# zju-vipa/ProtoPFormer

Measured on NVIDIA B200. Metric: prototype_head_train_images_per_sec, higher is better.
Workload: dtype bf16x3 split, fp32 accumulate (fp32-grade)

## Files before the change

include/protohead.h:

```cpp
#ifndef PROTOHEAD_B200_H
#define PROTOHEAD_B200_H

#include <stdint.h>

#ifdef __cplusplus
extern "C" {
#endif

#define PPH_VERSION 202

#define PPH_EINVAL   (-1)
#define PPH_EUNSUP   (-2)
#define PPH_EDRIVER  (-3)

#define PPH_MODE_FP32_FMA 0
#define PPH_MODE_BF16X3   1
#define PPH_MODE_BF16     2

#define PPH_ACT_LOG    0
#define PPH_ACT_LINEAR 1

typedef void* pph_stream_t;

int         pph_version(void);
// ... 63 lines not shown
                  int B, int N, int Din, int D, int K, void* workspace, int parts,
                  float* dWa, float* dba, float* dtokens, pph_stream_t stream);

int pph_loss_tail(const float* logits, const int64_t* labels, const float* ppc_losses,
                  float cov_coe, float mean_coe, float upstream, int B, int C,
                  float* partial, uint32_t* counter, float* out_losses, float* dlogits, pph_stream_t stream);

int pph_loss_combine(const float* ce_losses, const float* ppc_losses, float cov_coe, float mean_coe,
                     float* out_losses, pph_stream_t stream);

#define PPH_FUSE_MEAN 0
#define PPH_FUSE_MAX  1
#define PPH_FUSE_MIN  2
int pph_rollout_ws_bytes(int L, int B, int T, int k_discard, long long* bytes );
int pph_rollout_scores(const float* const* attn_layers , int L, int B, int H, int T,
                       int k_discard, int head_fusion, float identity_w, const float* v0, int drop_first,
                       void* workspace, float* scores, int K, int32_t* idx32, int64_t* idx64, pph_stream_t stream);

int pph_adamw_step(int n_seg, float* const* params, const float* const* grads, float* const* exp_avg,
                   float* const* exp_avg_sq, const long long* numel , const int* group ,
                   const float* hyper, double beta1, double beta2, float eps, float grad_scale,
                   int* step_state, pph_stream_t stream);

int pph_rollout_cls_rows(const float* const* cls_layers , int n_cls, int B, int H,
                         int Tc, int k_discard, int head_fusion, float identity_w, float* v0, pph_stream_t stream);

int pph_class_maps(const float* Zs, const float* z2s, const float* Pl, const float* p2l,
                   const int32_t* idx32, const int64_t* labels, int B, int K, int D, int P, int m, int N,
                   int act_fn, float eps, float* maps, pph_stream_t stream);


int pph_head_prep_supported(int B, int N, int Din, int D, int K);
int pph_head_prep(const float* scores, const float* tokens, const float* Wa, const float* ba,
                  int B, int H, int N, int Din, int D, int K, float center,
                  int32_t* idx32, int64_t* idx64,
                  float* Zs, float* Zc, float* z2s, float* z2c, float* z2s_ctr, float* z2c_ctr,
                  float* z2s_hi, float* z2c_hi, uint16_t* Zs_hi, uint16_t* Zs_lo, uint16_t* Zc_hi, uint16_t* Zc_lo,
                  const float* Pl, int P, uint16_t* Pl_hi, uint16_t* Pl_lo, float* p2l, float* p2l_ctr, float* p2l_hi,
                  const float* Pgl, int Pg, uint16_t* Pg_hi, uint16_t* Pg_lo, float* p2g, float* p2g_ctr, float* p2g_hi,
                  pph_stream_t stream);

int pph_head_mid_ws_bytes(int B, int K, int D, int P, int Pg, int C, int m, long long* bytes );
int pph_head_mid(const float* act_l, const float* act_g, const float* dmin_l, const float* dmin_g,
                 const int32_t* argmin_l, const float* Wl, const float* Wg, const int64_t* labels,
                 int B, int K, int D, int P, int Pg, int C, int m, int N,
                 float global_coe, int act_fn, float eps, float upstream, int train,
                 int use_ppc, const float* Zs, const float* z2s, const float* Pl, const float* p2l,
                 const int32_t* idx32, float cov_thresh, float mean_thresh, float cov_coe, float mean_coe,
                 void* workspace, void* bwd_workspace,
                 float* logits, float* logits_g, float* logits_l, float* losses, float* dlogits,
                 float* g_l, float* g_g, float* pairT, float* dZs_ppc, float* dP_img,
                 float* losses_mirror ,
                 pph_stream_t stream);

#define PPH_BWD2_TOKENS 1
#define PPH_BWD2_PROTOS 2
#define PPH_BWD2_CLS    4
int pph_similarity_bwd2_supported(int B, int K, int D, int P, int Pg);
int pph_similarity_bwd2_ws_bytes(int B, int K, int D, int P, long long* bytes );
int pph_similarity_bwd2(int parts, const float* g_l, const float* g_g, const float* pairT, void* bwd_workspace,
                        const float* Zs, const float* Zc, const float* Pl, const float* Pgl,
                        int B, int K, int D, int P, int Pg, int m,
                        const float* add_dZs, const float* dP_img, int dpre_out,
                        float* dZs, float* dZc, float* dPl, float* dPg, pph_stream_t stream);

int pph_similarity_bwd_fused(int parts ,
                             const float* g_l, const float* g_g, const int32_t* argmin_l,
                             const float* Zs, const float* Zc, const float* Pl, const float* Pgl,
                             int B, int K, int D, int P, int Pg, int m, void* workspace, void* step_workspace,
                             const float* add_dZs, const float* dP_img, int dpre_out,
                             float* dZs, float* dZc, float* dPl, float* dPg, pph_stream_t stream);

int pph_addon_bwd2_supported(int B, int N, int Din, int D, int K);
int pph_addon_bwd2_ws_bytes(int B, int N, int Din, int D, int K, long long* bytes );
int pph_addon_bwd2(int parts, const float* tokens, const int32_t* idx32, const float* Wa,
                   const float* dpre_s, const float* dpre_c,
                   int B, int N, int Din, int D, int K, void* workspace,
                   float* dWa, float* dba, float* dtokens, pph_stream_t stream);

int pph_addon_tc2_supported(int B, int N, int Din, int D, int K);
int pph_addon_tc2_ws_bytes(int B, int N, int Din, int D, int K, long long* bytes );
int pph_addon_fwd2(const float* tokens, const int32_t* idx32, const float* Wa, const float* ba,
                   int B, int N, int Din, int D, int K,
                   float* Zs, float* Zc, float* z2s, float* z2c,
                   float center, float* z2s_ctr, float* z2c_ctr, float* z2s_hi, float* z2c_hi,
                   uint16_t* Zs_hi, uint16_t* Zs_lo, uint16_t* Zc_hi, uint16_t* Zc_lo,
                   void* workspace, pph_stream_t stream);
int pph_select_addon_fwd(const float* scores , int H, const float* tokens, const float* Wa, const float* ba,
                         int B, int N, int Din, int D, int K, int32_t* idx32 ,
                         float* Zs, float* Zc, float* z2s, float* z2c,
                         float center, float* z2s_ctr, float* z2c_ctr, float* z2s_hi, float* z2c_hi,
                         uint16_t* Zs_hi, uint16_t* Zs_lo, uint16_t* Zc_hi, uint16_t* Zc_lo,
                         void* workspace, pph_stream_t stream);
int pph_addon_bwd3(int parts, const float* tokens, const int32_t* idx32, const float* Wa,
                   const float* dpre_s, const float* dpre_c, const float* dpre_add_s ,
                   int B, int N, int Din, int D, int K, void* workspace,
                   float* dWa, float* dba, float* dtokens, pph_stream_t stream);

int pph_ppc_dense_fwd(const float* act, const int32_t* idx32, const int64_t* labels, int B, int P, int K, int m, int N,
                      float cov_thresh, float mean_thresh, float* stats, float* partial, unsigned int* counter,
                      float* losses, pph_stream_t stream);
int pph_ppc_dense_bwd(const float* act, const int32_t* idx32, const int64_t* labels, const float* stats,
                      const float* g_cov, const float* g_mean, int B, int P, int K, int m, int N, float mean_thresh,
                      float* dact, pph_stream_t stream);

int pph_gather_rows_host(const float* tokens_host, const int32_t* idx32, int B, int N, int Din, int K,
// ... 12 lines not shown
```

protopformer_b200/_lib.py:

```python
from __future__ import annotations

import ctypes as C
import os

import torch

_HERE = os.path.dirname(os.path.abspath(__file__))
LIB_PATH = os.path.join(_HERE, "lib", "libprotohead_b200.so")

MODE_FP32_FMA, MODE_BF16X3, MODE_BF16 = 0, 1, 2
MODES = {"fp32_fma": MODE_FP32_FMA, "fp32": MODE_BF16X3, "bf16x3": MODE_BF16X3, "bf16": MODE_BF16}
ACT_LOG, ACT_LINEAR = 0, 1
ACTS = {"log": ACT_LOG, "linear": ACT_LINEAR}

_p, _i, _f = C.c_void_p, C.c_int, C.c_float

SIGNATURES = {
    "pph_version": [],
    "pph_last_error_string": [],
    "pph_sm_count": [],
    "pph_set_option": [C.c_char_p, _i],
    "pph_select_topk": [_p, _i, _i, _i, _i, _p, _p, _p],
    "pph_addon_fwd": [_p, _p, _p, _p, _i, _i, _i, _i, _i, _p, _p, _p, _p, _f, _p, _p, _p, _p, _p, _p, _p, _p, _p],
    "pph_split_rows": [_p, _i, _i, _f, _p, _p, _p, _p, _p, _p],
    "pph_similarity_fwd": [_i, _i, _f, _i, _i, _i, _i, _i] + [_p] * 24,
    "pph_similarity_plan": [_i, _i, _i, _i, _i, _i, _i, C.POINTER(C.c_int), C.POINTER(C.c_int)],
    "pph_logits_fwd": [_p, _p, _p, _p, _i, _i, _i, _i, _f, _p, _p, _p, _p],
    "pph_ppc_fwd": [_p, _p, _p, _p, _p, _p, _i, _i, _i, _i, _i, _i, _i, _f, _f, _f, _p, _p, _p, _p, _p, _p],
    "pph_ppc_bwd": [_p, _p, _p, _p, _p, _p, _p, _f, _f, _i, _i, _i, _i, _i, _i, _i, _f, _f, _f, _i, _p, _p, _p],
    "pph_logits_bwd": [_p, _p, _p, _p, _p, _p, _p, _i, _i, _i, _i, _f, _i, _f, _p, _p, _p],
    "pph_similarity_bwd_ws_bytes": [_i, _i, _i, _i, _i, C.POINTER(C.c_longlong)],
    "pph_similarity_bwd": [_p, _p, _p, _p, _p, _p, _p, _i, _i, _i, _i, _i, _p, _i, _p, _p, _p, _p, _p, _p, _p],
    "pph_loss_tail": [_p, _p, _p, _f, _f, _f, _i, _i, _p, _p, _p, _p, _p],
    "pph_loss_combine": [_p, _p, _f, _f, _p, _p],
    "pph_rollout_ws_bytes": [_i, _i, _i, _i, C.POINTER(C.c_longlong)],
    "pph_rollout_scores": [_p, _i, _i, _i, _i, _i, _i, _f, _p, _i, _p, _p, _i, _p, _p, _p],
    "pph_adamw_step": [_i, _p, _p, _p, _p, _p, _p, _p, C.c_double, C.c_double, _f, _f, _p, _p],
    "pph_rollout_cls_rows": [_p, _i, _i, _i, _i, _i, _i, _f, _p, _p],
    "pph_class_maps": [_p, _p, _p, _p, _p, _p, _i, _i, _i, _i, _i, _i, _i, _f, _p, _p],
    "pph_addon_bwd_ws_bytes": [_i, _i, _i, _i, _i, C.POINTER(C.c_longlong)],
    "pph_addon_bwd": [_p, _p, _p, _p, _p, _p, _p, _i, _i, _i, _i, _i, _p, _i, _p, _p, _p, _p],
    "pph_head_prep_supported": [_i, _i, _i, _i, _i],
    "pph_head_prep": [_p, _p, _p, _p, _i, _i, _i, _i, _i, _i, _f] + [_p] * 14 + [_p, _i, _p, _p, _p, _p, _p] * 2 + [_p],
    "pph_head_mid_ws_bytes": [_i, _i, _i, _i, _i, _i, _i, C.POINTER(C.c_longlong)],
    "pph_head_mid": [_p] * 8 + [_i] * 8 + [_f, _i, _f, _f, _i, _i] + [_p] * 5 + [_f] * 4 + [_p] * 14,
    "pph_similarity_bwd2_supported": [_i, _i, _i, _i, _i],
    "pph_similarity_bwd2_ws_bytes": [_i, _i, _i, _i, C.POINTER(C.c_longlong)],
    "pph_similarity_bwd2": [_i] + [_p] * 8 + [_i] * 6 + [_p, _p, _i] + [_p] * 5,
    "pph_addon_bwd2_supported": [_i, _i, _i, _i, _i],
    "pph_addon_bwd2_ws_bytes": [_i, _i, _i, _i, _i, C.POINTER(C.c_longlong)],
    "pph_addon_bwd2": [_i] + [_p] * 5 + [_i] * 5 + [_p] * 5,
    "pph_similarity_bwd_fused": [_i] + [_p] * 7 + [_i] * 6 + [_p, _p, _p, _p, _i] + [_p] * 5,
    "pph_addon_tc2_supported": [_i, _i, _i, _i, _i],
    "pph_addon_tc2_ws_bytes": [_i, _i, _i, _i, _i, C.POINTER(C.c_longlong)],
    "pph_addon_fwd2": [_p, _p, _p, _p, _i, _i, _i, _i, _i, _p, _p, _p, _p, _f] + [_p] * 10,
    "pph_addon_bwd3": [_i] + [_p] * 6 + [_i] * 5 + [_p] * 5,
    "pph_select_addon_fwd": [_p, _i, _p, _p, _p, _i, _i, _i, _i, _i, _p, _p, _p, _p, _p, _f] + [_p] * 10,
    "pph_ppc_dense_fwd": [_p, _p, _p, _i, _i, _i, _i, _i, _f, _f, _p, _p, _p, _p, _p],
    "pph_ppc_dense_bwd": [_p, _p, _p, _p, _p, _p, _i, _i, _i, _i, _i, _f, _p, _p],
    "pph_gather_rows_host": [_p, _p, _i, _i, _i, _i, _p, _i, _p],
    "pph_peer_flag_bytes": [C.POINTER(C.c_longlong)],
    "pph_peer_allreduce": [_p, C.c_ulonglong, C.c_longlong, _i, _i, C.c_longlong, C.c_longlong, _i, _i, _p],
}
_RESTYPES = {"pph_last_error_string": C.c_char_p}

KERNELS_PER_CALL = {
    "pph_select_topk": 1, "pph_addon_fwd": 1, "pph_split_rows": 1, "pph_logits_fwd": 1, "pph_ppc_fwd": 1,
    "pph_ppc_bwd": 1, "pph_logits_bwd": 1, "pph_similarity_bwd": 2, "pph_addon_bwd": 3, "pph_loss_tail": 1, "pph_loss_combine": 1, "pph_rollout_scores": 2, "pph_adamw_step": 1, "pph_class_maps": 1, "pph_rollout_cls_rows": 1,
    "pph_head_prep": 1, "pph_head_mid": 1, "pph_similarity_bwd_fused": 1, "pph_addon_bwd2": 1, "pph_addon_fwd2": 1,
    "pph_peer_allreduce": 1, "pph_gather_rows_host": 1,
    "pph_ppc_dense_fwd": 1, "pph_ppc_dense_bwd": 1, "pph_select_addon_fwd": 1,
}

_ENV_OPTIONS = {"PPH_PDL": "pdl", "PPH_SIM_LANES": "sim_lanes", "PPH_SIM_SHARED": "sim_shared", "PPH_SIM_EPI": "sim_epi",
                "PPH_ROLLOUT": "rollout", "PPH_CLASSMAP": "classmap", "PPH_DEBUG": "debug",
                "PPH_LOGITS_BWD": "logits_bwd", "PPH_GATHER": "gather"}

_lib = None
_launches = 0


def launch_count() -> int:
    return _launches


def load() -> C.CDLL:
    global _lib
    if _lib is None:
        if not os.path.exists(LIB_PATH):
            raise RuntimeError(
                f"{LIB_PATH} is missing: build it with `python -m protopformer_b200.build` "
                "(needs nvcc; there is no CPU or PyTorch fallback for the prototype head)")
        lib = C.CDLL(LIB_PATH)
        for name, args in SIGNATURES.items():
            fn = getattr(lib, name)
            fn.argtypes = args
            fn.restype = _RESTYPES.get(name, C.c_int)
        for env, opt in _ENV_OPTIONS.items():
            v = os.environ.get(env)
            if v is not None and v.strip() != "":
                if lib.pph_set_option(opt.encode(), int(v)) != 0:
                    raise RuntimeError(f"{env}: {lib.pph_last_error_string().decode()}")
        _lib = lib
    return _lib


_DTYPES = (torch.float32, torch.int32, torch.int64, torch.bfloat16, torch.uint8, torch.int8, torch.uint16, torch.int16)


def _ptr(t):
    if t is None:
        return None
    assert t.is_cuda, "prototype-head tensors must live on a CUDA device (no CPU path exists)"
    assert t.is_contiguous(), "prototype-head tensors must be contiguous"
    assert t.dtype in _DTYPES, f"prototype-head entry points do not take {t.dtype} tensors (cast to float32 first)"
    return t.data_ptr()


def _stream():
    return torch.cuda.current_stream().cuda_stream


# ... 22 lines not shown
```

protopformer_b200/csrc/pph_mid.cu:

```cuda
#include <math.h>

#include "pph_bins.cuh"
#include "pph_common.cuh"
#include "pph_step2.cuh"

namespace pph {

constexpr int kMidThreads = 256;
constexpr int kMidTB = 64;
constexpr int kMidPS = 32;
constexpr int kMidAST = 68;

struct MidArgs {
    int B, Bp, K, D, P, Pg, C, Cp, m, N, side;
    int tiles_b, S_l, S_g, nsl_l, nsl_g;
    int n_ll, n_bin, n_ppc, n_cls_cta;
    int have_ppc;
    int ppc_dpre;
    float gc, eps, upstream, cov_thresh, mean_thresh, cov_coe, mean_coe;
    int act_fn, train;
    const float *act_l, *act_g, *dmin_l, *dmin_g;
    const int32_t* argmin_l;
    const float *Wl, *Wg;
    const int64_t* labels;
    float *logits, *logits_g, *logits_l, *losses, *dlogits, *g_l, *g_g;
    float* losses_mirror;
    float2* pairT;
    float *part, *dlT, *ce_part, *ppc_part, *ppc_losses;
    unsigned int* ctr;
    int32_t *bin_start, *item_start, *bin_list;
    int4* item_desc;
    int32_t *cls_id, *cls_start, *cls_item, *cls_order;
    const float *Zs, *z2s, *Pl, *p2l;
    const int32_t* idx;
    float *dZs_ppc, *dP_img;
};

__device__ __forceinline__ float block_sum_any(float v, float* red, int nwarp) {
    v = warp_sum(v);
    const int lane = threadIdx.x & 31, warp = threadIdx.x >> 5;
    __syncthreads();
    if (lane == 0) red[warp] = v;
    __syncthreads();
    float s = 0.f;
    for (int w = 0; w < nwarp; ++w) s += red[w];
    return s;
}

__device__ __forceinline__ float block_sum_mid(float v, float* red) {
    v = warp_sum(v);
    const int lane = threadIdx.x & 31, warp = threadIdx.x >> 5;
    __syncthreads();
    if (lane == 0) red[warp] = v;
    __syncthreads();
    float s = 0.f;
#pragma unroll
    for (int w = 0; w < kMidThreads / 32; ++w) s += red[w];
    return s;
}

__device__ __forceinline__ void write_total(const MidArgs& a) {
    const float ce = __ldcg(a.losses + 1);
    const float cov = a.have_ppc ? __ldcg(a.ppc_losses) : 0.f, mean = a.have_ppc ? __ldcg(a.ppc_losses + 1) : 0.f;
    const float total = ce + a.cov_coe * cov + a.mean_coe * mean;
    a.losses[0] = total;
    a.losses[2] = cov;
    a.losses[3] = mean;
    if (a.losses_mirror) {
        *reinterpret_cast<float4*>(a.losses_mirror) = make_float4(total, ce, cov, mean);
        __threadfence_system();
    }
}
__device__ __forceinline__ void role_finished(const MidArgs& a) {
    if (!a.have_ppc) {
        write_total(a);
        return;
    }
    __threadfence();
    if (atomicAdd(a.ctr + 2, 1u) == 1u) {
        __threadfence();
        write_total(a);
        a.ctr[2] = 0u;
// ... 182 lines not shown
        }
        cp_async_commit();
        const bool keepW = nsl <= Sg;
        const float coef = glob ? a.gc : 1.0f - a.gc;
        const float* dmin = glob ? a.dmin_g : a.dmin_l;
        float* gout = glob ? a.g_g : a.g_l;
        for (int sl = sg; sl < nsl; sl += Sg) {
            const int p0 = sl * kMidPS;
            if (!keepW) {
                __syncthreads();
                stage_w(Ws, W, np, p0, C, WST);
                cp_async_commit();
            }
            cp_async_wait<0>();
            __syncthreads();
            float g8[8];
#pragma unroll
            for (int i = 0; i < 8; ++i) g8[i] = 0.f;
#pragma unroll 4
            for (int c = 0; c < C; ++c) {
                const float4 d0 = *reinterpret_cast<const float4*>(&dls[c * kMidAST + warp * 8]);
                const float4 d1 = *reinterpret_cast<const float4*>(&dls[c * kMidAST + warp * 8 + 4]);
                const float w = Ws[lane * WST + c];
                g8[0] = fmaf(d0.x, w, g8[0]); g8[1] = fmaf(d0.y, w, g8[1]); g8[2] = fmaf(d0.z, w, g8[2]); g8[3] = fmaf(d0.w, w, g8[3]);
                g8[4] = fmaf(d1.x, w, g8[4]); g8[5] = fmaf(d1.y, w, g8[5]); g8[6] = fmaf(d1.z, w, g8[6]); g8[7] = fmaf(d1.w, w, g8[7]);
            }
            const int p = p0 + lane;
            if (p < np) {
                float2 pr[8];
#pragma unroll
                for (int i = 0; i < 8; ++i) {
                    const int b = b0 + warp * 8 + i;
                    float g = 0.f;
                    int am = 0;
                    if (b < B) {
                        const size_t o = (size_t)b * np + p;
                        g = coef * g8[i] * dact_of_dist(__ldg(dmin + o), a.act_fn, a.eps);
                        gout[o] = g;
                        am = glob ? a.K : __ldg(a.argmin_l + o);
                    }
                    pr[i] = make_float2(g, __int_as_float(am));
                }
                if (a.pairT) {
                    float4* dst = reinterpret_cast<float4*>(a.pairT + (size_t)(glob ? a.P + p : p) * a.Bp + b0 + warp * 8);
#pragma unroll
                    for (int i = 0; i < 4; ++i) dst[i] = make_float4(pr[2 * i].x, pr[2 * i].y, pr[2 * i + 1].x, pr[2 * i + 1].y);
                }
            }
        }
    }
    grid_finish(a.ctr, a.ctr + 1, (unsigned int)a.n_ll);
}

__device__ __forceinline__ void ppc_role(const MidArgs& a, int b, int part, int nsplit, float* sm) {
    const int nthr = blockDim.x;
    const int K = a.K, D = a.D, m = a.m, B = a.B, side = a.side;
    const int zs = D + 4;
    float* Prow = sm;
    float* Zt = Prow + m * D;
    float* dsl = Zt + (size_t)K * zs;
    float* wbuf = dsl + m * K;
    float* st = wbuf + m * K;
    float* red = st + m * 8;
    const int tid = threadIdx.x, lane = tid & 31, warp = tid >> 5, nwarp = nthr >> 5;
    long y = a.labels[b];
    if (y < 0) y = 0;
    if (y * m + m > a.P) y = a.P / m - 1;
    const int prow0 = (int)y * m;
    for (int i = tid; i < m * D / 4; i += nthr) cp_async16(Prow + 4 * i, a.Pl + (size_t)prow0 * D + 4 * i);
    const float* Zb = a.Zs + (size_t)b * K * D;
    {
        const int d4 = D >> 2;
        for (int r = warp; r < K; r += nwarp)
            for (int c = lane; c < d4; c += 32) cp_async16(Zt + (size_t)r * zs + 4 * c, Zb + (size_t)r * D + 4 * c);
    }
    cp_async_commit();
    cp_async_wait<0>();
    __syncthreads();
    const int JG = K * m <= nthr ? m : (K * 5 <= nthr ? 5 : (K * 3 <= nthr ? 3 : (K * 2 <= nthr ? 2 : 1)));
    for (int t = tid; t < K * JG; t += nthr) {
        const int r = t % K, jg = t / K;
        const float4* zr = reinterpret_cast<const float4*>(Zt + (size_t)r * zs);
        const float zz = __ldg(a.z2s + (size_t)b * K + r);
        for (int j = jg; j < m; j += JG) {
            const float4* pr = reinterpret_cast<const float4*>(Prow + (size_t)j * D);
            float a0 = 0.f, a1 = 0.f, a2 = 0.f, a3 = 0.f;
#pragma unroll 4
            for (int c = 0; c < D / 4; ++c) {
                const float4 z = zr[c], p = pr[c];
                a0 = fmaf(z.x, p.x, a0); a1 = fmaf(z.y, p.y, a1); a2 = fmaf(z.z, p.z, a2); a3 = fmaf(z.w, p.w, a3);
            }
            const float dot = (a0 + a1) + (a2 + a3);
            const float d = relu_keep_nan(zz + fmaf(-2.0f, dot, __ldg(a.p2l + prow0 + j)));
            dsl[j * K + r] = d;
            wbuf[j * K + r] = act_of_dist(d, a.act_fn, a.eps);
        }
    }
    __syncthreads();
    float cov_sum = 0.f;
    const float scale = (float)a.N / (float)(a.N - 1);
    for (int j = warp; j < m; j += nwarp) {
        float S = 0.f, Sr = 0.f, Sc = 0.f;
        for (int k = lane; k < K; k += 32) {
            const float w = wbuf[j * K + k];
            const int n = __ldg(a.idx + (size_t)b * K + k);
            S += w;
// ... 75 lines not shown
        const float dw = (dV * ((dr * dr - Vr) + (dc * dc - Vc)) + st[j * 8 + 6] * dr + st[j * 8 + 7] * dc) / S;
        const float d = dsl[j * K + r];
        dsl[j * K + r] = 2.0f * dw * dact_of_dist(d, a.act_fn, a.eps);
    }
    __syncthreads();
    const int ngrp = (D + 127) >> 7;
    for (int r = warp * nsplit + part; r < K; r += nwarp * nsplit) {
        float S = 0.f;
        for (int j = 0; j < m; ++j) S += dsl[j * K + r];
        float* out = a.dZs_ppc + ((size_t)b * K + r) * D;
        for (int g = 0; g < ngrp; ++g) {
            const int d = g * 128 + lane * 4;
            if (d >= D) continue;
            const float4 z = *reinterpret_cast<const float4*>(Zt + (size_t)r * zs + d);
            float4 acc = make_float4(z.x * S, z.y * S, z.z * S, z.w * S);
#pragma unroll 2
            for (int j = 0; j < m; ++j) {
                const float c = -dsl[j * K + r];
                const float4 p = *reinterpret_cast<const float4*>(Prow + j * D + d);
                acc.x = fmaf(c, p.x, acc.x); acc.y = fmaf(c, p.y, acc.y); acc.z = fmaf(c, p.z, acc.z); acc.w = fmaf(c, p.w, acc.w);
            }
            if (a.ppc_dpre) {
                acc.x *= z.x * (1.0f - z.x); acc.y *= z.y * (1.0f - z.y); acc.z *= z.z * (1.0f - z.z); acc.w *= z.w * (1.0f - z.w);
            }
            *reinterpret_cast<float4*>(out + d) = acc;
        }
    }
    for (int it = warp * nsplit + part; it < m * ngrp; it += nwarp * nsplit) {
        const int j = it / ngrp, g = it - j * ngrp;
        const int d = g * 128 + lane * 4;
        if (d >= D) continue;
        float S = 0.f;
        float4 acc = make_float4(0.f, 0.f, 0.f, 0.f);
#pragma unroll 4
        for (int r = 0; r < K; ++r) {
            const float c = dsl[j * K + r];
            const float4 z = *reinterpret_cast<const float4*>(Zt + (size_t)r * zs + d);
            S += c;
            acc.x = fmaf(c, z.x, acc.x); acc.y = fmaf(c, z.y, acc.y); acc.z = fmaf(c, z.z, acc.z); acc.w = fmaf(c, z.w, acc.w);
        }
        const float4 p = *reinterpret_cast<const float4*>(Prow + j * D + d);
        *reinterpret_cast<float4*>(a.dP_img + ((size_t)b * m + j) * D + d) =
            make_float4(p.x * S - acc.x, p.y * S - acc.y, p.z * S - acc.z, p.w * S - acc.w);
    }
}

template <int CJ>
__global__ void __launch_bounds__(kMidThreads)
head_mid_kernel(const MidArgs a) {
    pdl_sync();
    extern __shared__ __align__(16) float sm_mid[];
    const int bid = blockIdx.x;
    if (bid < a.n_ll) {
        ll_role<CJ>(a, sm_mid);
    } else if (bid < a.n_ll + a.n_bin) {
        bin_tokens_body<false>(bid - a.n_ll, a.argmin_l, a.K, a.P, a.bin_start, a.item_start, a.bin_list,
                        reinterpret_cast<int*>(sm_mid), a.item_desc);
    } else if (bid < a.n_ll + a.n_bin + a.n_ppc) {
        ppc_role(a, bid - a.n_ll - a.n_bin, 0, 1, sm_mid);
    } else {
        const int n_cls = a.P / a.m;
        for (int b = threadIdx.x; b < a.B; b += kMidThreads) {
            long y = a.labels[b];
            if (y < 0) y = 0;
            if (y * a.m + a.m > a.P) y = a.P / a.m - 1;
            a.cls_id[b] = (int)y;
        }
        __threadfence();
        __syncthreads();
        bin_tokens_body<true>(0, a.cls_id, n_cls, a.B, a.cls_start, a.cls_item, a.cls_order, reinterpret_cast<int*>(sm_mid));
    }
}

constexpr int kPpcSplit = 2, kPpcThreads = 512;
__global__ void __launch_bounds__(kPpcThreads)
head_ppc_kernel(const MidArgs a) {
    pdl_sync();
    extern __shared__ __align__(16) float sm_mid[];
    ppc_role(a, blockIdx.x / kPpcSplit, blockIdx.x % kPpcSplit, kPpcSplit, sm_mid);
}

struct MidPlan {
    int tiles_b, nsl_l, nsl_g, S_l, S_g, n_ll, Cp, Bp;
    size_t smem_ll, smem_ppc, smem_bin;
};

static MidPlan mid_plan(int B, int K, int D, int P, int Pg, int C, int m, int max_ctas) {
    MidPlan p;
    p.tiles_b = ceil_div(B, kMidTB);
    p.nsl_l = ceil_div(P, kMidPS);
    p.nsl_g = Pg > 0 ? ceil_div(Pg, kMidPS) : 0;
    p.Cp = (C + 3) & ~3;
    p.Bp = p.tiles_b * kMidTB;
    int budget = max_ctas / p.tiles_b;
    const int need = Pg > 0 ? 2 : 1;
    if (budget < need) budget = need;
    if (p.nsl_l + p.nsl_g <= budget) {
        p.S_l = p.nsl_l;
        p.S_g = p.nsl_g;
    } else if (Pg > 0) {
        p.S_l = (int)((long)budget * p.nsl_l / (p.nsl_l + p.nsl_g));
        if (p.S_l < 1) p.S_l = 1;
        if (p.S_l > budget - 1) p.S_l = budget - 1;
        p.S_g = budget - p.S_l;
        if (p.S_l > p.nsl_l) p.S_l = p.nsl_l;
        if (p.S_g > p.nsl_g) p.S_g = p.nsl_g;
    } else {
        p.S_l = budget < p.nsl_l ? budget : p.nsl_l;
        p.S_g = 0;
    }
    p.n_ll = p.tiles_b * (p.S_l + p.S_g);
    const int WST = C | 1;
    p.smem_ll = sizeof(float) * ((size_t)kMidPS * WST + (size_t)kMidPS * kMidAST + (size_t)C * kMidAST + 2 * 4 * 64 * 4 + 3 * 256 + 8);
    p.smem_ppc = sizeof(float) * ((size_t)m * D + (size_t)K * (D + 4) + 2 * (size_t)m * K + 8 * (size_t)m + 32);
    p.smem_bin = bin_tokens_smem_bytes(K);
    return p;
}

struct MidWs {
    unsigned int* ctr;
    float *part, *dlT, *ce_part, *ppc_part, *ppc_losses;
    size_t bytes;
};

static MidWs mid_carve(void* base, const MidPlan& p, int B) {
    MidWs w;
    char* q = static_cast<char*>(base);
    size_t off = 0;
    auto take = [&](size_t n) { char* r = q ? q + off : nullptr; off += (n + 255) / 256 * 256; return r; };
    w.ctr = reinterpret_cast<unsigned int*>(take(sizeof(int) * 8));
    w.ppc_losses = reinterpret_cast<float*>(take(sizeof(float) * 2));
    w.ce_part = reinterpret_cast<float*>(take(sizeof(float) * (size_t)B));
    w.ppc_part = reinterpret_cast<float*>(take(sizeof(float) * 2 * (size_t)B));
    w.dlT = reinterpret_cast<float*>(take(sizeof(float) * (size_t)p.Cp * p.Bp));
    w.part = reinterpret_cast<float*>(take(sizeof(float) * (size_t)(p.S_l + p.S_g) * B * p.Cp));
    w.bytes = off + 256;
    return w;
}

static int mid_max_ctas() {
    int n = pph_sm_count();
    return n > 0 ? n : 148;
}

}

extern "C" int pph_head_mid_ws_bytes(int B, int K, int D, int P, int Pg, int C, int m, long long* bytes) {
    using namespace pph;
    PPH_REQUIRE(bytes && B >= 1 && K >= 1 && D >= 1 && P >= 1 && Pg >= 0 && C >= 1 && m >= 1, PPH_EINVAL,
                "pph_head_mid_ws_bytes: bad args");
    const MidPlan p = mid_plan(B, K, D, P, Pg, C, m, 1 << 20);
    *bytes = (long long)mid_carve(nullptr, p, B).bytes;
    return 0;
}

extern "C" int pph_head_mid(const float* act_l, const float* act_g, const float* dmin_l, const float* dmin_g,
                            const int32_t* argmin_l, const float* Wl, const float* Wg, const int64_t* labels,
                            int B, int K, int D, int P, int Pg, int C, int m, int N,
                            float global_coe, int act_fn, float eps, float upstream, int train,
                            int use_ppc, const float* Zs, const float* z2s, const float* Pl, const float* p2l,
                            const int32_t* idx32, float cov_thresh, float mean_thresh, float cov_coe, float mean_coe,
                            void* workspace, void* bwd_workspace,
                            float* logits, float* logits_g, float* logits_l, float* losses, float* dlogits,
                            float* g_l, float* g_g, float* pairT, float* dZs_ppc, float* dP_img,
                            float* losses_mirror, pph_stream_t stream) {
    using namespace pph;
    PPH_REQUIRE(act_l && dmin_l && Wl && labels && workspace && logits && logits_g && logits_l && losses, PPH_EINVAL,
                "pph_head_mid: null pointer");
    PPH_REQUIRE(Pg == 0 || (act_g && dmin_g && Wg), PPH_EINVAL, "pph_head_mid: null global-branch pointer");
    PPH_REQUIRE((reinterpret_cast<uintptr_t>(losses_mirror) & 15) == 0, PPH_EINVAL, "pph_head_mid: losses_mirror must be 16-byte aligned");
    PPH_REQUIRE(B >= 1 && K >= 1 && D >= 4 && P >= 1 && Pg >= 0 && C >= 1 && m >= 1 && N >= 2, PPH_EINVAL,
                "pph_head_mid: bad dims");
    PPH_REQUIRE(C <= 256, PPH_EUNSUP, "pph_head_mid: C=%d > 256 (use the modular entry points)", C);
    PPH_REQUIRE(!train || (argmin_l && dlogits && g_l && bwd_workspace && (Pg == 0 || g_g)), PPH_EINVAL,
                "pph_head_mid: null training pointer");
    PPH_REQUIRE(!use_ppc || (Zs && z2s && Pl && p2l && idx32 && (!train || (dZs_ppc && dP_img))), PPH_EINVAL,
                "pph_head_mid: null PPC pointer");
    const int max_ctas = mid_max_ctas();
    const MidPlan p = mid_plan(B, K, D, P, Pg, C, m, max_ctas);
    const MidWs w = mid_carve(workspace, p, B);
    MidArgs a;
    a.B = B; a.Bp = p.Bp; a.K = K; a.D = D; a.P = P; a.Pg = Pg; a.C = C; a.Cp = p.Cp; a.m = m; a.N = N;
    a.side = (int)lrint(sqrt((double)N));
    a.tiles_b = p.tiles_b; a.S_l = p.S_l; a.S_g = p.S_g; a.nsl_l = p.nsl_l; a.nsl_g = p.nsl_g;
    a.ppc_dpre = (use_ppc & 4) ? 1 : 0;
    use_ppc &= 3;
    const bool have_ppc = use_ppc != 0, run_ll = use_ppc != 3, run_ppc = use_ppc == 1 || use_ppc == 3;
    a.have_ppc = have_ppc ? 1 : 0;
    a.n_ll = run_ll ? p.n_ll : 0;
    a.n_bin = (train && run_ll) ? B : 0;
    a.n_ppc = run_ppc ? B : 0;
    a.gc = global_coe; a.eps = eps; a.upstream = upstream; a.cov_thresh = cov_thresh; a.mean_thresh = mean_thresh;
    a.cov_coe = cov_coe; a.mean_coe = mean_coe; a.act_fn = act_fn; a.train = train;
    a.act_l = act_l; a.act_g = act_g; a.dmin_l = dmin_l; a.dmin_g = dmin_g; a.argmin_l = argmin_l;
    a.Wl = Wl; a.Wg = Wg; a.labels = labels;
    a.logits = logits; a.logits_g = logits_g; a.logits_l = logits_l; a.losses = losses; a.dlogits = dlogits;
    a.losses_mirror = losses_mirror;
    a.g_l = g_l; a.g_g = g_g; a.pairT = reinterpret_cast<float2*>(pairT);
    a.part = w.part; a.dlT = w.dlT; a.ce_part = w.ce_part; a.ppc_part = w.ppc_part; a.ppc_losses = w.ppc_losses;
    a.ctr = w.ctr;
    a.bin_start = a.item_start = a.bin_list = nullptr;
    a.item_desc = nullptr;
    a.cls_id = a.cls_start = a.cls_item = a.cls_order = nullptr;
    a.n_cls_cta = 0;
    if (train) {
        const Step2Bins bw = carve_bins(bwd_workspace, B, K, P);
        a.bin_start = bw.bin_start; a.item_start = bw.item_start; a.bin_list = bw.bin_list;
        a.item_desc = bw.item_desc;
        a.cls_id = bw.cls_id; a.cls_start = bw.cls_start; a.cls_item = bw.cls_item; a.cls_order = bw.cls_order;
        if (have_ppc && run_ll && bin_tokens_smem_bytes(P / m) <= 200 * 1024) a.n_cls_cta = 1;
    }
    a.Zs = Zs; a.z2s = z2s; a.Pl = Pl; a.p2l = p2l; a.idx = idx32; a.dZs_ppc = dZs_ppc; a.dP_img = dP_img;
    size_t smem = run_ll ? p.smem_ll : 0;
    if (a.n_bin && p.smem_bin > smem) smem = p.smem_bin;
    if (a.n_cls_cta && bin_tokens_smem_bytes(P / m) > smem) smem = bin_tokens_smem_bytes(P / m);
    if (have_ppc) {
        PPH_REQUIRE(D % 4 == 0 && a.side * a.side == N && P >= m && m <= kMidThreads, PPH_EINVAL, "pph_head_mid: bad PPC dims");
        PPH_REQUIRE(p.smem_ppc <= 200 * 1024, PPH_EUNSUP, "pph_head_mid: an image's K x D slice does not fit shared memory");
        if (run_ppc && p.smem_ppc > smem) smem = p.smem_ppc;
    }
    PPH_REQUIRE(smem <= 220 * 1024, PPH_EUNSUP, "pph_head_mid: shared memory %zu B", smem);
    PPH_REQUIRE(p.n_ll <= max_ctas, PPH_EUNSUP, "pph_head_mid: B=%d needs %d co-resident CTAs (> %d SMs)", B, p.n_ll,
                max_ctas);
    if (use_ppc == 3) {
        cudaError_t e = opt_in_smem(head_ppc_kernel, (int)p.smem_ppc);
        if (e != cudaSuccess) { set_error("pph_head_mid: %s", cudaGetErrorString(e)); return (int)e; }
        launch_k(head_ppc_kernel, dim3(B * kPpcSplit), dim3(kPpcThreads), p.smem_ppc, as_stream(stream), a);
        return launch_status("pph_head_mid(ppc)");
    }
    const int cj = ceil_div(C, 32);
    PPH_REQUIRE(!(have_ppc && train && run_ll) || a.n_cls_cta == 1, PPH_EUNSUP, "pph_head_mid: too many classes");

    const dim3 grid(a.n_ll + a.n_bin + a.n_ppc + a.n_cls_cta), block(kMidThreads);
    cudaStream_t st = as_stream(stream);
#define PPH_MID(CJ)                                                                                                   \
    do {                                                                                                              \
        cudaError_t e = opt_in_smem(head_mid_kernel<CJ>, (int)smem); \
        if (e != cudaSuccess) { set_error("pph_head_mid: %s", cudaGetErrorString(e)); return (int)e; }                \
        launch_k(head_mid_kernel<CJ>, grid, block, smem, st, a);                                                      \
    } while (0)
    if (cj <= 4) PPH_MID(4);
    else if (cj <= 7) PPH_MID(7);
    else PPH_MID(8);
#undef PPH_MID
    return launch_status("pph_head_mid");
}
```

protopformer_b200/ops.py:

```python
from __future__ import annotations

import dataclasses
import math

import torch

from . import _lib


@dataclasses.dataclass(frozen=True)
class HeadConfig:

    K: int
    global_coe: float = 0.5
    act_fn: str = "log"
    eps: float = 1e-4
    mode: str = "fp32"
    ppc_cov_thresh: float = 1.0
    ppc_mean_thresh: float = 2.0
    center: float = 0.5

    @property
    def mode_id(self) -> int:
        return _lib.MODES[self.mode]
# ... 593 lines not shown

class FusedHeadStep:

    def __init__(self, cfg: HeadConfig, B, N, Din, D, P, Pg, C, m, device, heads: int = 0, ppc_cov_coe: float = 0.1,
                 ppc_mean_coe: float = 0.5, train: bool = True, use_ppc: bool = True, schedule=None, variants=None):
        if not fused_step_supported(B, N, Din, D, cfg.K, P, Pg, C, m):
            raise ValueError("shape outside FusedHeadStep's kernels: use FusedHeadStepV1")
        self.cfg, self.train, self.use_ppc = cfg, train, use_ppc
        tc_bits = _lib.load().pph_addon_tc2_supported(B, N, Din, D, cfg.K)
        tc1_ok = Din % 8 == 0 and D % 8 == 0 and cfg.mode_id != _lib.MODE_FP32_FMA
        v = {"prep": "tc" if (tc_bits & 1) else ("tc1" if tc1_ok else "simt"),
             "addon_bwd": "tc" if (tc_bits & 6) == 6 else "simt", "bwd": "gather", "ppc": "late",
             "select": "fused" if (tc_bits & 8) else "kernel"}
        v.update(variants or {})
        if v["select"] == "fused" and not (tc_bits & 8):
            v["select"] = "kernel"
        if v["prep"] == "tc" and not (tc_bits & 1):
            v["prep"] = "tc1" if tc1_ok else "simt"
        if v["prep"] == "tc1" and not tc1_ok:
            v["prep"] = "simt"
        if v["addon_bwd"] == "tc" and (tc_bits & 6) != 6:
            v["addon_bwd"] = "simt"
        if v["bwd"] == "staged" and not _lib.load().pph_similarity_bwd2_supported(B, cfg.K, D, P, Pg):
            v["bwd"] = "gather"
        self.variants = v
        self.stop_after = 0
        self.dims = (B, N, Din, D, P, Pg, C, m, heads)
        self.cov_coe, self.mean_coe = float(ppc_cov_coe), float(ppc_mean_coe)
        K = cfg.K
        f32, bf, i32 = torch.float32, torch.bfloat16, torch.int32
        e = lambda *s, dt=f32: torch.empty(s, dtype=dt, device=device)
        self.split = cfg.mode_id != _lib.MODE_FP32_FMA
        self.idx32 = e(B, K, dt=i32)
        self.Zs, self.Zc, self.z2s, self.z2c = e(B, K, D), e(B, D), e(B, K), e(B)
        names = ("z2s_ctr", "z2c_ctr", "z2s_hi", "z2c_hi", "Zs_hi", "Zs_lo", "Zc_hi", "Zc_lo", "P_hi", "P_lo", "Pg_hi",
                 "Pg_lo", "p2_ctr", "p2_hi", "pg2_ctr", "pg2_hi")
        if self.split:
            shapes = ((B, K), (B,), (B, K), (B,), (B * K, D), (B * K, D), (B, D), (B, D), (P, D), (P, D), (Pg, D), (Pg, D),
                      (P,), (P,), (Pg,), (Pg,))
            for n, sh in zip(names, shapes):
                setattr(self, n, e(*sh, dt=bf if ("_hi" in n or "_lo" in n) and n[0] in "ZP" else f32))
        else:
            for n in names:
                setattr(self, n, None)
        self.p2, self.pg2 = e(P), e(Pg)
        self.dmin_l, self.act_l, self.argmin = e(B, P), e(B, P), e(B, P, dt=i32)
        self.dmin_g, self.act_g = e(B, Pg), e(B, Pg)
        self.logits, self.logits_g, self.logits_l = e(B, C), e(B, C), e(B, C)
        self.losses = torch.zeros(4, dtype=f32, device=device)
        self.ws_mid = _ws("pph_head_mid_ws_bytes", B, K, D, P, Pg, C, m, zero=True, device=device)
        self.ws_tc = _ws("pph_addon_tc2_ws_bytes", B, N, Din, D, K, zero=True, device=device)
        self.side = torch.cuda.Stream(device=device)
        self.side2 = torch.cuda.Stream(device=device)
        self.ev = [torch.cuda.Event() for _ in range(8)]
        self.dlogits = self.g_l = self.g_g = self.pairT = self.ws_bins = None
        self.dZs_ppc = self.dP_img = None
        if train:
            Bp = (B + 63) // 64 * 64
            self.dlogits, self.g_l, self.g_g = e(B, C), e(B, P), e(B, Pg)
            self.pairT = e(P + Pg, Bp, 2)
            self.ws_bins = _ws("pph_similarity_bwd2_ws_bytes", B, K, D, P, zero=True, device=device)
            self.ws_gather = bwd_workspace(B, K, D, P, Pg, device)
            if use_ppc:
                self.dZs_ppc, self.dP_img = e(B, K, D), e(B, m, D)
            self.dZs, self.dZc = e(B, K, D), e(B, D)
            self.dtokens = e(B, 1 + N, Din)
            self.ws_addon = _ws("pph_addon_bwd2_ws_bytes", B, N, Din, D, K, zero=True, device=device)
            if self.variants["addon_bwd"] == "tc":
                self.dtokens.zero_()


    def step(self, tokens, scores, labels, Wa, ba, P, Pg, Wl, Wg, grads=None, upstream: float = 1.0, reduce_hook=None,
             idx32=None, loss_mirror=None):
        own_idx = self.idx32
        sel_idx = own_idx if idx32 is None else idx32
        B, N, Din, D, Pn, Pgn, C, m, H = self.dims
        cfg, K = self.cfg, self.cfg.K
        c = _lib.call
        main, side, side2, ev = torch.cuda.current_stream(), self.side, self.side2, self.ev
        hook = reduce_hook or (lambda which: None)
        if self.variants["prep"] in ("tc", "tc1"):
            ev[3].record(main)
            side.wait_event(ev[3])
            with torch.cuda.stream(side):
                c("pph_split_rows", P, Pn, D, float(cfg.center), self.P_hi, self.P_lo, self.p2, self.p2_ctr, self.p2_hi)
                c("pph_split_rows", Pg, Pgn, D, float(cfg.center), self.Pg_hi, self.Pg_lo, self.pg2, self.pg2_ctr, self.pg2_hi)
                if self.train and self.variants["addon_bwd"] == "tc":
                    self.dtokens.zero_()
                ev[4].record(side)
            if self.variants["prep"] == "tc1":
                if idx32 is None:
                    c("pph_select_topk", scores, B, max(H, 1), N, K, sel_idx, None)
                c("pph_addon_fwd", tokens, sel_idx, Wa, ba, B, N, Din, D, K, self.Zs, self.Zc, self.z2s, self.z2c,
                  float(cfg.center), self.z2s_ctr, self.z2c_ctr, self.z2s_hi, self.z2c_hi, self.Zs_hi, self.Zs_lo,
                  self.Zc_hi, self.Zc_lo)
            elif idx32 is None and self.variants["select"] == "fused":
                c("pph_select_addon_fwd", scores, max(H, 1), tokens, Wa, ba, B, N, Din, D, K, sel_idx, self.Zs, self.Zc,
                  self.z2s, self.z2c, float(cfg.center), self.z2s_ctr, self.z2c_ctr, self.z2s_hi, self.z2c_hi, self.Zs_hi,
                  self.Zs_lo, self.Zc_hi, self.Zc_lo, self.ws_tc)
            else:
                if idx32 is None:
                    c("pph_select_topk", scores, B, max(H, 1), N, K, sel_idx, None)
                c("pph_addon_fwd2", tokens, sel_idx, Wa, ba, B, N, Din, D, K, self.Zs, self.Zc, self.z2s, self.z2c,
                  float(cfg.center), self.z2s_ctr, self.z2c_ctr, self.z2s_hi, self.z2c_hi, self.Zs_hi, self.Zs_lo,
                  self.Zc_hi, self.Zc_lo, self.ws_tc)
            main.wait_event(ev[4])
        else:
            if self.train and self.variants["addon_bwd"] == "tc":
                ev[3].record(main)
                side.wait_event(ev[3])
                with torch.cuda.stream(side):
                    self.dtokens.zero_()
                    ev[4].record(side)
            c("pph_head_prep", scores, tokens, Wa, ba, B, max(H, 1), N, Din, D, K, float(cfg.center), sel_idx, None,
              self.Zs, self.Zc, self.z2s, self.z2c, self.z2s_ctr, self.z2c_ctr, self.z2s_hi, self.z2c_hi,
              self.Zs_hi, self.Zs_lo, self.Zc_hi, self.Zc_lo,
              P, Pn, self.P_hi, self.P_lo, self.p2, self.p2_ctr, self.p2_hi,
              Pg, Pgn, self.Pg_hi, self.Pg_lo, self.pg2, self.pg2_ctr, self.pg2_hi)
            if self.train and self.variants["addon_bwd"] == "tc":
                main.wait_event(ev[4])
        if self.stop_after == 1:
            return self.losses
        mode = cfg.mode_id
        sel = {_lib.MODE_FP32_FMA: 0, _lib.MODE_BF16X3: 1, _lib.MODE_BF16: 2}[mode]
        c("pph_similarity_fwd", mode, cfg.act_id, float(cfg.eps), B, K, D, Pn, Pgn, self.Zs, self.Zc,
          (self.z2s, self.z2s_ctr, self.z2s_hi)[sel], (self.z2c, self.z2c_ctr, self.z2c_hi)[sel],
          self.Zs_hi, self.Zs_lo, self.Zc_hi, self.Zc_lo, P, Pg,
          (self.p2, self.p2_ctr, self.p2_hi)[sel], (self.pg2, self.pg2_ctr, self.pg2_hi)[sel],
          self.P_hi, self.P_lo, self.Pg_hi, self.Pg_lo,
          self.dmin_l, self.argmin, self.act_l, self.dmin_g, self.act_g, None, None)
        if self.stop_after == 2:
            return self.losses
        ppc = self.use_ppc and self.train
        vr = self.variants
        late = ppc and vr["ppc"] == "late" and vr["bwd"] == "gather" and vr["addon_bwd"] == "tc"
        split_ppc = ppc and (vr["ppc"] == "split" or late)

        def mid(use_ppc):
            c("pph_head_mid", self.act_l, self.act_g, self.dmin_l, self.dmin_g, self.argmin, Wl, Wg, labels,
              B, K, D, Pn, Pgn, C, m, N, float(cfg.global_coe), cfg.act_id, float(cfg.eps), float(upstream),
              1 if self.train else 0, use_ppc, self.Zs, self.z2s, P, self.p2, sel_idx,
              float(cfg.ppc_cov_thresh), float(cfg.ppc_mean_thresh), self.cov_coe, self.mean_coe,
              self.ws_mid, self.ws_bins, self.logits, self.logits_g, self.logits_l, self.losses, self.dlogits,
              self.g_l, self.g_g, self.pairT if vr["bwd"] == "staged" else None, self.dZs_ppc if ppc else None,
              self.dP_img if ppc else None, loss_mirror)

        if split_ppc:
            ev[0].record(main)
            side.wait_event(ev[0])
            with torch.cuda.stream(side):
                mid(3 + (4 if late else 0))
                ev[6 if late else 1].record(side)
            mid(2)
            if not late:
                main.wait_event(ev[1])
        else:
            mid(1 if ppc else 0)
        if not self.train or self.stop_after == 3:
            if late:
                main.wait_event(ev[6])
            return self.losses

        def gather(parts, add, dpi):
            c("pph_similarity_bwd_fused", parts, self.g_l, self.g_g, self.argmin, self.Zs, self.Zc, P, Pg, B, K, D, Pn, Pgn,
              m, self.ws_gather, self.ws_bins, add, dpi, 1, self.dZs, self.dZc, grads["P"], grads["Pg"])

        dpre_add = None
        if late:
            gather(3, None, None)
            ev[2].record(main)
            with torch.cuda.stream(side):
                side.wait_event(ev[2])
                gather(4, None, self.dP_img)
                hook("protos")
                ev[1].record(side)
            dpre_add = self.dZs_ppc
        elif vr["bwd"] == "gather":
            gather(3, self.dZs_ppc if ppc else None, self.dP_img if ppc else None)
            hook("protos")
            ev[1].record(main)
        else:
            bwd = lambda parts: c("pph_similarity_bwd2", parts, self.g_l, self.g_g, self.pairT, self.ws_bins, self.Zs,
                                  self.Zc, P, Pg, B, K, D, Pn, Pgn, m, self.dZs_ppc if ppc else None,
# ... 48 lines not shown
```

Measured before the change: 428,200.

## Detect class-structured last layer and use closed-form logits and grads

Adds a kernel on the side stream that checks, on every call, whether each last-layer weight matrix takes only two values: one for a prototype's own class and another everywhere else. When both matrices match, the mid kernel's logits role computes logits as a per-class sum plus a total sum, and computes prototype gradients in closed form instead of through the general matrix path. Otherwise it falls back to the existing role. The check costs an extra kernel launch, a full read of the weights and an event wait before the mid stage, and it only pays off when the weights keep this structure.

```diff
diff --git a/include/protohead.h b/include/protohead.h
--- a/include/protohead.h
+++ b/include/protohead.h
@@ -139,6 +139,9 @@
                  float* g_l, float* g_g, float* pairT, float* dZs_ppc, float* dP_img,
                  float* losses_mirror ,
                  pph_stream_t stream);
+
+#define PPH_LL_PATTERN_BYTES 32
+int pph_last_layer_pattern(const float* Wl, int P, const float* Wg, int Pg, int C, void* workspace, pph_stream_t stream);
 
 #define PPH_BWD2_TOKENS 1
 #define PPH_BWD2_PROTOS 2
diff --git a/protopformer_b200/_lib.py b/protopformer_b200/_lib.py
--- a/protopformer_b200/_lib.py
+++ b/protopformer_b200/_lib.py
@@ -44,6 +44,7 @@
     "pph_head_prep": [_p, _p, _p, _p, _i, _i, _i, _i, _i, _i, _f] + [_p] * 14 + [_p, _i, _p, _p, _p, _p, _p] * 2 + [_p],
     "pph_head_mid_ws_bytes": [_i, _i, _i, _i, _i, _i, _i, C.POINTER(C.c_longlong)],
     "pph_head_mid": [_p] * 8 + [_i] * 8 + [_f, _i, _f, _f, _i, _i] + [_p] * 5 + [_f] * 4 + [_p] * 14,
+    "pph_last_layer_pattern": [_p, _i, _p, _i, _i, _p, _p],
     "pph_similarity_bwd2_supported": [_i, _i, _i, _i, _i],
     "pph_similarity_bwd2_ws_bytes": [_i, _i, _i, _i, C.POINTER(C.c_longlong)],
     "pph_similarity_bwd2": [_i] + [_p] * 8 + [_i] * 6 + [_p, _p, _i] + [_p] * 5,
@@ -67,7 +68,7 @@
 KERNELS_PER_CALL = {
     "pph_select_topk": 1, "pph_addon_fwd": 1, "pph_split_rows": 1, "pph_logits_fwd": 1, "pph_ppc_fwd": 1,
     "pph_ppc_bwd": 1, "pph_logits_bwd": 1, "pph_similarity_bwd": 2, "pph_addon_bwd": 3, "pph_loss_tail": 1, "pph_loss_combine": 1, "pph_rollout_scores": 2, "pph_adamw_step": 1, "pph_class_maps": 1, "pph_rollout_cls_rows": 1,
-    "pph_head_prep": 1, "pph_head_mid": 1, "pph_similarity_bwd_fused": 1, "pph_addon_bwd2": 1, "pph_addon_fwd2": 1,
+    "pph_head_prep": 1, "pph_head_mid": 1, "pph_last_layer_pattern": 1, "pph_similarity_bwd_fused": 1, "pph_addon_bwd2": 1, "pph_addon_fwd2": 1,
     "pph_peer_allreduce": 1, "pph_gather_rows_host": 1,
     "pph_ppc_dense_fwd": 1, "pph_ppc_dense_bwd": 1, "pph_select_addon_fwd": 1,
 }
diff --git a/protopformer_b200/csrc/pph_mid.cu b/protopformer_b200/csrc/pph_mid.cu
--- a/protopformer_b200/csrc/pph_mid.cu
+++ b/protopformer_b200/csrc/pph_mid.cu
@@ -1,4 +1,6 @@
 #include <math.h>
+
+#include <algorithm>
 
 #include "pph_bins.cuh"
 #include "pph_common.cuh"
@@ -10,6 +12,17 @@
 constexpr int kMidTB = 64;
 constexpr int kMidPS = 32;
 constexpr int kMidAST = 68;
+
+struct LLPattern {
+    int ok;
+    float a, b;
+    int unused;
+};
+struct LLPatternWs {
+    LLPattern rec[2];
+    unsigned int bad, ticket;
+};
+static_assert(sizeof(LLPattern) * 2 == PPH_LL_PATTERN_BYTES, "protohead.h documents two 16-byte records");
 
 struct MidArgs {
     int B, Bp, K, D, P, Pg, C, Cp, m, N, side;
@@ -28,6 +41,7 @@
     float2* pairT;
     float *part, *dlT, *ce_part, *ppc_part, *ppc_losses;
     unsigned int* ctr;
+    LLPatternWs* pattern;
     int32_t *bin_start, *item_start, *bin_list;
     int4* item_desc;
     int32_t *cls_id, *cls_start, *cls_item, *cls_order;
@@ -316,6 +330,117 @@
     grid_finish(a.ctr, a.ctr + 1, (unsigned int)a.n_ll);
 }
 
+__device__ __forceinline__ float block_max_mid(float v, float* red) {
+#pragma unroll
+    for (int o = 16; o > 0; o >>= 1) v = fmaxf(v, __shfl_xor_sync(0xffffffffu, v, o));
+    const int lane = threadIdx.x & 31, warp = threadIdx.x >> 5;
+    __syncthreads();
+    if (lane == 0) red[warp] = v;
+    __syncthreads();
+    float s = red[0];
+#pragma unroll
+    for (int w = 1; w < kMidThreads / 32; ++w) s = fmaxf(s, red[w]);
+    return s;
+}
+
+__device__ __forceinline__ void ll_class_grad(const MidArgs& a, int b, bool glob, const LLPattern& w, float Sdl,
+                                              const float* dls) {
+    const int np = glob ? a.Pg : a.P, m = np / a.C;
+    const float coef = glob ? a.gc : 1.0f - a.gc;
+    const float* dmin = glob ? a.dmin_g : a.dmin_l;
+    float* gout = glob ? a.g_g : a.g_l;
+    const float bS = w.b * Sdl, amb = w.a - w.b;
+    const size_t row = (size_t)b * np;
+    constexpr int U = 4;
+    for (int p0 = threadIdx.x; p0 < np; p0 += U * kMidThreads) {
+        float d[U];
+#pragma unroll
+        for (int u = 0; u < U; ++u) {
+            const int p = p0 + u * kMidThreads;
+            d[u] = p < np ? __ldg(dmin + row + p) : 0.f;
+        }
+#pragma unroll
+        for (int u = 0; u < U; ++u) {
+            const int p = p0 + u * kMidThreads;
+            if (p >= np) break;
+            const float g = coef * fmaf(amb, dls[p / m], bS) * dact_of_dist(d[u], a.act_fn, a.eps);
+            gout[row + p] = g;
+            if (a.pairT)
+                a.pairT[(size_t)(glob ? a.P + p : p) * a.Bp + b] =
+                    make_float2(g, __int_as_float(glob ? a.K : __ldg(a.argmin_l + row + p)));
+        }
+    }
+}
+
+__device__ void ll_class_role(const MidArgs& a, const LLPattern& wl, const LLPattern& wg, float* sm) {
+    const int tid = threadIdx.x, c = tid;
+    const int B = a.B, C = a.C, ml = a.P / C, mg = a.Pg / C;
+    float* dls = sm;
+    float* zs = dls + kMidThreads;
+    float* red = zs + kMidThreads;
+    const float kl = (1.0f - a.gc) * (wl.a - wl.b), kg = a.gc * (wg.a - wg.b);
+    for (int b = blockIdx.x; b < B; b += a.n_ll) {
+        float sl = 0.f, sg = 0.f;
+        if (c < C) {
+            const float* rl = a.act_l + (size_t)b * a.P + (size_t)c * ml;
+            const float* rg = a.act_g + (size_t)b * a.Pg + (size_t)c * mg;
+            for (int j = 0; j < ml; ++j) sl += __ldg(rl + j);
+            for (int j = 0; j < mg; ++j) sg += __ldg(rg + j);
+        }
+        const float Tl = block_sum_mid(sl, red), Tg = block_sum_mid(sg, red);
+        const float z = c < C ? fmaf(kl, sl, kg * sg) : -INFINITY;
+        zs[c] = z;
+        if (c < C) {
+            const float lv = fmaf(wl.a - wl.b, sl, wl.b * Tl), gv = fmaf(wg.a - wg.b, sg, wg.b * Tg);
+            a.logits_l[(size_t)b * C + c] = lv;
+            a.logits_g[(size_t)b * C + c] = gv;
+            a.logits[(size_t)b * C + c] = a.gc * gv + (1.0f - a.gc) * lv;
+        }
+        const float mx = block_max_mid(z, red);
+        const float e = c < C ? expf(z - mx) : 0.f;
+        const float se = block_sum_mid(e, red);
+        long y = a.labels[b];
+        if (y < 0) y = 0;
+        if (y >= C) y = C - 1;
+        if (tid == 0) a.ce_part[b] = logf(se) + mx - zs[y];
+        if (a.train) {
+            const float dl = c < C ? (e / se - (c == (int)y ? 1.0f : 0.0f)) * (a.upstream / (float)B) : 0.f;
+            if (c < C) a.dlogits[(size_t)b * C + c] = dl;
+            dls[c] = dl;
+            const float Sdl = block_sum_mid(dl, red);
+            ll_class_grad(a, b, false, wl, Sdl, dls);
+            ll_class_grad(a, b, true, wg, Sdl, dls);
+        }
+        __syncthreads();
+    }
+    if (a.train && a.pairT) {
+        for (int b = a.B + blockIdx.x; b < a.Bp; b += a.n_ll)
+            for (int p = tid; p < a.P + a.Pg; p += kMidThreads) a.pairT[(size_t)p * a.Bp + b] = make_float2(0.f, 0.f);
+    }
+    __shared__ int last;
+    __syncthreads();
+    if (tid == 0) {
+        __threadfence();
+        last = atomicAdd(a.ctr + 4, 1u) == (unsigned int)a.n_ll - 1u;
+        if (last) {
+            __threadfence();
+            a.pattern->rec[0].ok = 0;
+            a.pattern->rec[1].ok = 0;
+            a.ctr[4] = 0u;
+        }
+    }
+    __syncthreads();
+    if (last) {
+        float v = 0.f;
+        for (int i = tid; i < B; i += kMidThreads) v += __ldcg(a.ce_part + i);
+        const float ce = block_sum_mid(v, red) / (float)B;
+        if (tid == 0) {
+            a.losses[1] = ce;
+            role_finished(a);
+        }
+    }
+}
+
 __device__ __forceinline__ void ppc_role(const MidArgs& a, int b, int part, int nsplit, float* sm) {
     const int nthr = blockDim.x;
     const int K = a.K, D = a.D, m = a.m, B = a.B, side = a.side;
@@ -497,7 +622,9 @@
     extern __shared__ __align__(16) float sm_mid[];
     const int bid = blockIdx.x;
     if (bid < a.n_ll) {
-        ll_role<CJ>(a, sm_mid);
+        const LLPattern wl = a.pattern->rec[0], wg = a.pattern->rec[1];
+        if (wl.ok && wg.ok) ll_class_role(a, wl, wg, sm_mid);
+        else ll_role<CJ>(a, sm_mid);
     } else if (bid < a.n_ll + a.n_bin) {
         bin_tokens_body<false>(bid - a.n_ll, a.argmin_l, a.K, a.P, a.bin_start, a.item_start, a.bin_list,
                         reinterpret_cast<int*>(sm_mid), a.item_desc);
@@ -563,6 +690,7 @@
 }
 
 struct MidWs {
+    LLPatternWs* pattern;
     unsigned int* ctr;
     float *part, *dlT, *ce_part, *ppc_part, *ppc_losses;
     size_t bytes;
@@ -573,6 +701,7 @@
     char* q = static_cast<char*>(base);
     size_t off = 0;
     auto take = [&](size_t n) { char* r = q ? q + off : nullptr; off += (n + 255) / 256 * 256; return r; };
+    w.pattern = reinterpret_cast<LLPatternWs*>(take(sizeof(LLPatternWs)));
     w.ctr = reinterpret_cast<unsigned int*>(take(sizeof(int) * 8));
     w.ppc_losses = reinterpret_cast<float*>(take(sizeof(float) * 2));
     w.ce_part = reinterpret_cast<float*>(take(sizeof(float) * (size_t)B));
@@ -588,6 +717,78 @@
     return n > 0 ? n : 148;
 }
 
+constexpr int kPatThreads = 256, kPatVecPerThread = 4;
+
+__device__ __forceinline__ unsigned int pattern_scan(const float* __restrict__ W, int C, int n, bool vec4) {
+    if (n == 0) return 0u;
+    if (n % C != 0) return 1u;
+    const int m = n / C, total = C * n;
+    const float a = __ldg(W), b = C > 1 ? __ldg(W + n) : a;
+    const int t0 = blockIdx.x * blockDim.x + threadIdx.x, stride = gridDim.x * blockDim.x;
+    bool bad = false;
+    if (vec4) {
+        const float4* W4 = reinterpret_cast<const float4*>(W);
+#pragma unroll 4
+        for (int i = t0; i < total / 4; i += stride) {
+            const float4 v = __ldg(W4 + i);
+            const int e = 4 * i, c = e / n, p = e - c * n;
+            bad |= v.x != ((p / m == c) ? a : b);
+            bad |= v.y != (((p + 1) / m == c) ? a : b);
+            bad |= v.z != (((p + 2) / m == c) ? a : b);
+            bad |= v.w != (((p + 3) / m == c) ? a : b);
+        }
+    } else {
+#pragma unroll 4
+        for (int e = t0; e < total; e += stride) {
+            const int c = e / n, p = e - c * n;
+            bad |= __ldg(W + e) != ((p / m == c) ? a : b);
+        }
+    }
+    return bad ? 1u : 0u;
+}
+
+__device__ __forceinline__ LLPattern pattern_record(const float* W, int C, int n, bool bad) {
+    LLPattern r;
+    r.ok = !bad;
+    r.a = n > 0 ? W[0] : 0.f;
+    r.b = n > 0 ? (C > 1 ? W[n] : r.a) : 0.f;
+    r.unused = 0;
+    return r;
+}
+
+__global__ void __launch_bounds__(kPatThreads)
+last_layer_pattern_kernel(const float* __restrict__ Wl, int P, int vec_l, const float* __restrict__ Wg, int Pg, int vec_g,
+                          int C, LLPatternWs* ws) {
+    pdl_sync();
+    const unsigned int bits = pattern_scan(Wl, C, P, vec_l) | (pattern_scan(Wg, C, Pg, vec_g) << 1);
+    const int bad_l = __syncthreads_or(bits & 1u), bad_g = __syncthreads_or(bits & 2u);
+    if (threadIdx.x != 0) return;
+    if (bad_l || bad_g) atomicOr(&ws->bad, (bad_l ? 1u : 0u) | (bad_g ? 2u : 0u));
+    __threadfence();
+    if (atomicAdd(&ws->ticket, 1u) != gridDim.x - 1u) return;
+    __threadfence();
+    const unsigned int all = atomicExch(&ws->bad, 0u);
+    ws->rec[0] = pattern_record(Wl, C, P, all & 1u);
+    ws->rec[1] = pattern_record(Wg, C, Pg, all & 2u);
+    ws->ticket = 0u;
+}
+
+}
+
+extern "C" int pph_last_layer_pattern(const float* Wl, int P, const float* Wg, int Pg, int C, void* workspace,
+                                      pph_stream_t stream) {
+    using namespace pph;
+    PPH_REQUIRE(Wl && workspace && (Pg == 0 || Wg), PPH_EINVAL, "pph_last_layer_pattern: null pointer");
+    PPH_REQUIRE(P >= 1 && Pg >= 0 && C >= 1, PPH_EINVAL, "pph_last_layer_pattern: bad dims");
+    PPH_REQUIRE((long long)C * P < (1LL << 31) && (long long)C * Pg < (1LL << 31), PPH_EUNSUP,
+                "pph_last_layer_pattern: C x P = %lld entries", (long long)C * (P > Pg ? P : Pg));
+    auto vec4 = [](const float* W, int n) { return (n % 4 == 0 && (reinterpret_cast<uintptr_t>(W) & 15) == 0) ? 1 : 0; };
+    const int vl = vec4(Wl, P), vg = vec4(Wg, Pg);
+    const int per_cta = kPatThreads * kPatVecPerThread * 4;
+    const int ctas = std::min(mid_max_ctas(), std::max(1, ceil_div(C * std::max(P, Pg), per_cta)));
+    launch_k(last_layer_pattern_kernel, dim3(ctas), dim3(kPatThreads), 0, as_stream(stream), Wl, P, vl, Wg, Pg, vg, C,
+             static_cast<LLPatternWs*>(workspace));
+    return launch_status("pph_last_layer_pattern");
 }
 
 extern "C" int pph_head_mid_ws_bytes(int B, int K, int D, int P, int Pg, int C, int m, long long* bytes) {
@@ -644,6 +845,7 @@
     a.g_l = g_l; a.g_g = g_g; a.pairT = reinterpret_cast<float2*>(pairT);
     a.part = w.part; a.dlT = w.dlT; a.ce_part = w.ce_part; a.ppc_part = w.ppc_part; a.ppc_losses = w.ppc_losses;
     a.ctr = w.ctr;
+    a.pattern = w.pattern;
     a.bin_start = a.item_start = a.bin_list = nullptr;
     a.item_desc = nullptr;
     a.cls_id = a.cls_start = a.cls_item = a.cls_order = nullptr;
diff --git a/protopformer_b200/ops.py b/protopformer_b200/ops.py
--- a/protopformer_b200/ops.py
+++ b/protopformer_b200/ops.py
@@ -669,7 +669,7 @@
         self.ws_tc = _ws("pph_addon_tc2_ws_bytes", B, N, Din, D, K, zero=True, device=device)
         self.side = torch.cuda.Stream(device=device)
         self.side2 = torch.cuda.Stream(device=device)
-        self.ev = [torch.cuda.Event() for _ in range(8)]
+        self.ev = [torch.cuda.Event() for _ in range(9)]
         self.dlogits = self.g_l = self.g_g = self.pairT = self.ws_bins = None
         self.dZs_ppc = self.dP_img = None
         if train:
@@ -696,6 +696,11 @@
         c = _lib.call
         main, side, side2, ev = torch.cuda.current_stream(), self.side, self.side2, self.ev
         hook = reduce_hook or (lambda which: None)
+
+        def last_layer_pattern():
+            c("pph_last_layer_pattern", Wl, Pn, Wg, Pgn, C, self.ws_mid)
+            ev[8].record(side)
+
         if self.variants["prep"] in ("tc", "tc1"):
             ev[3].record(main)
             side.wait_event(ev[3])
@@ -705,6 +710,7 @@
                 if self.train and self.variants["addon_bwd"] == "tc":
                     self.dtokens.zero_()
                 ev[4].record(side)
+                last_layer_pattern()
             if self.variants["prep"] == "tc1":
                 if idx32 is None:
                     c("pph_select_topk", scores, B, max(H, 1), N, K, sel_idx, None)
@@ -723,12 +729,13 @@
                   self.Zc_hi, self.Zc_lo, self.ws_tc)
             main.wait_event(ev[4])
         else:
-            if self.train and self.variants["addon_bwd"] == "tc":
-                ev[3].record(main)
-                side.wait_event(ev[3])
-                with torch.cuda.stream(side):
+            ev[3].record(main)
+            side.wait_event(ev[3])
+            with torch.cuda.stream(side):
+                if self.train and self.variants["addon_bwd"] == "tc":
                     self.dtokens.zero_()
                     ev[4].record(side)
+                last_layer_pattern()
             c("pph_head_prep", scores, tokens, Wa, ba, B, max(H, 1), N, Din, D, K, float(cfg.center), sel_idx, None,
               self.Zs, self.Zc, self.z2s, self.z2c, self.z2s_ctr, self.z2c_ctr, self.z2s_hi, self.z2c_hi,
               self.Zs_hi, self.Zs_lo, self.Zc_hi, self.Zc_lo,
@@ -737,6 +744,7 @@
             if self.train and self.variants["addon_bwd"] == "tc":
                 main.wait_event(ev[4])
         if self.stop_after == 1:
+            main.wait_event(ev[8])
             return self.losses
         mode = cfg.mode_id
         sel = {_lib.MODE_FP32_FMA: 0, _lib.MODE_BF16X3: 1, _lib.MODE_BF16: 2}[mode]
@@ -746,6 +754,7 @@
           (self.p2, self.p2_ctr, self.p2_hi)[sel], (self.pg2, self.pg2_ctr, self.pg2_hi)[sel],
           self.P_hi, self.P_lo, self.Pg_hi, self.Pg_lo,
           self.dmin_l, self.argmin, self.act_l, self.dmin_g, self.act_g, None, None)
+        main.wait_event(ev[8])
         if self.stop_after == 2:
             return self.losses
         ppc = self.use_ppc and self.train
```

Measured after the change: 457,800, median of 6. 6.9% higher.
